# carsonmw3/wavelet-compression

Hardware: AMD Instinct MI355X
Metric: fp64 cells/s, fwd transform+threshold+pack, keep=0.999 (higher is better)
Workload: dtype f64; 1 GPU; c2: 1024 x 64^3 fp64 boxes per GPU, 1 component, keep 0.999, wc_forward (payload bytes identical to the reference's serialize()); boxes_per_gpu=1024, global_batch=1024, parallelism=box-sharded x1

## Files before the change

wavelet-compression_amd/csrc/wc_capi.cpp:

```cpp
#include "wc_ctx.h"

#include <algorithm>
#include <cmath>
#include <cstring>
#include <string>
#include <vector>

using namespace wc;

namespace {

int stage_transform(wc_ctx* c, const void* d_cells, int dtype, double keep, bool sparse) {
    Plan& P = c->plan;
    const UnitDev* du = (const UnitDev*)P.d_units.p;
    const XTile* dxt = (const XTile*)P.d_xtiles.p;
    hipError_t e = hipSuccess;
    if ((e = hipMemsetAsync(c->state.p, 0, P.state_bytes, c->stream)) != hipSuccess)
        return hip_fail(c, e, "memset state");
    unsigned long long* key = (unsigned long long*)((uint8_t*)c->state.p + 16);
    const size_t n = P.units.size();
    uint32_t* spos = (uint32_t*)((uint8_t*)c->state.p + 16 + 12 * n);
    float* coef = (float*)c->coef.p;
    uint8_t* flags = sparse && P.any_sparse ? (uint8_t*)c->flags.p : nullptr;
    {
        StageTimer t(c, WC_STAGE_TRANSFORM);
        e = launch_transform(c->stream, d_cells, dtype, du, dxt, P.ngen, P.lds_gen, coef, 0, key);
        if (e == hipSuccess)
            e = launch_transform_fast(c->stream, d_cells, dtype, du, dxt + P.ngen, P.nfast, P.lds_fast, coef, 0,
                                      key, flags, spos, keep, persistent_grid(c, 0, P.lds_fast));
        if (e == hipSuccess && flags)
            e = launch_transform_fallback(c->stream, d_cells, dtype, du, (int)P.units.size(), dxt, P.lds_fast, coef,
                                          key, spos, keep);
    }
    c->sparse_staged = flags != nullptr;
    return e == hipSuccess ? WC_OK : hip_fail(c, e, "transform launch");
}

int stage_emit(wc_ctx* c, int n, double keep, const float* gthresh, uint8_t* d_payload, uint64_t* d_offsets,
               uint32_t* d_kept, uint2* d_rows = nullptr, const float* d_uthresh = nullptr) {
    Plan& P = c->plan;
    uint8_t* st = (uint8_t*)c->state.p;
    EmitParams p{};
    p.units = (const UnitDev*)P.d_units.p;
    p.edesc = (const EmitDesc*)P.d_edesc.p;
    p.n = n;
    p.ordered = use_ordered(c) ? (c->opt_reverse ? 2u : 1u) : 0u;
    p.key = (const unsigned long long*)(st + 16);
    p.tickets = (uint32_t*)(st + 16 + 8ull * n);
    p.status = (unsigned long long*)(st + round_up(16 + 20ull * n, 8));
    p.payload = d_payload;
    p.offsets = d_offsets;
    p.kept = d_kept;
    p.err = (uint32_t*)c->errflag.p;
    p.keep = keep;
    if (gthresh) {
        p.use_gthresh = 1;
        p.gthresh = *gthresh;
    }
    p.flags = (c->sparse_staged && !gthresh && !d_uthresh) ? (const uint8_t*)c->flags.p : nullptr;
    p.rowinfo = d_rows;
    p.uthresh = d_uthresh;
    StageTimer t(c, WC_STAGE_EMIT);
    hipError_t e = launch_emit(c->stream, p, (const float*)c->coef.p, P.nedesc_small,
                               (uint32_t)P.edesc.size() - P.nedesc_small);
    if (e != hipSuccess) return hip_fail(c, e, "emit launch");
    return WC_OK;
}

int forward_staged(wc_ctx* c, const void* d_cells, int dtype, int n, double keep, uint8_t* d_payload,
                   uint64_t* d_offsets, uint32_t* d_kept, uint2* d_rows = nullptr) {
    int rc = stage_transform(c, d_cells, dtype, keep, c->opt_sparse);
    return rc ? rc : stage_emit(c, n, keep, nullptr, d_payload, d_offsets, d_kept, d_rows);
}

int pin_begin(wc_ctx* c, size_t in_bytes, size_t dev_bytes, uint8_t** pin) {
    int rc;
    hipError_t e;
    if ((rc = ensure(c, c->tol_in, dev_bytes))) return rc;
    if (!c->tol_ev && (e = hipEventCreateWithFlags(&c->tol_ev, hipEventDisableTiming)) != hipSuccess)
        return hip_fail(c, e, "event");
    if (c->tol_ev_live && (e = hipEventSynchronize(c->tol_ev)) != hipSuccess) return hip_fail(c, e, "pinned upload");
    c->tol_ev_live = false;
    if (c->tol_pin_bytes < in_bytes) {
        if (c->tol_pin) (void)hipHostFree(c->tol_pin);
        c->tol_pin = nullptr;
        c->tol_pin_bytes = 0;
        const size_t want = std::max(in_bytes, size_t(4096));
        if ((e = hipHostMalloc(&c->tol_pin, want, hipHostMallocDefault)) != hipSuccess) {
            c->tol_pin = nullptr;
            return fail(c, WC_ERR_NOMEM, std::string("pinned block: ") + hipGetErrorString(e));
        }
        c->tol_pin_bytes = want;
    }
    *pin = (uint8_t*)c->tol_pin;
    return WC_OK;
}

int pin_upload(wc_ctx* c, size_t in_bytes) {
    hipError_t e;
    if ((e = hipMemcpyAsync(c->tol_in.p, c->tol_pin, in_bytes, hipMemcpyHostToDevice, c->stream)) != hipSuccess ||
        (e = hipEventRecord(c->tol_ev, c->stream)) != hipSuccess)
        return hip_fail(c, e, "pinned upload");
    c->tol_ev_live = true;
    return WC_OK;
}

int stage_tol(wc_ctx* c, int n, const double* tol, float* d_thresh, double* d_bound, const float** uthresh) {
    const Plan& P = c->plan;
    const uint32_t solo = (uint32_t)c->opt_tol_solo;
    const uint32_t chunk = std::min<uint32_t>(solo, 8);
    std::vector<uint32_t> slot(n), split;
    std::vector<uint2> items;
    for (int u = 0; u < n; ++u) {
        const uint32_t nt = P.units[u].nftiles;
        if (nt <= solo) {
            slot[u] = 0xffffffffu;
            continue;
        }
        slot[u] = (uint32_t)split.size();
        split.push_back((uint32_t)u);
        for (uint32_t t = 0; t < nt; t += chunk) items.push_back(make_uint2((uint32_t)u, t));
    }
    const size_t nsplit = split.size(), nitems = items.size();
    const size_t o_items = sizeof(double) * n, o_slot = o_items + sizeof(uint2) * nitems, o_split = o_slot + 4ull * n,
                 in_bytes = o_split + 4 * nsplit, o_thresh = round_up(in_bytes, 8);
    int rc;
    hipError_t e;
    uint8_t* pin = nullptr;
    if ((nsplit && (rc = ensure(c, c->tol_bins, sizeof(uint32_t) * WC_HIST_BINS * nsplit))) ||
        (rc = pin_begin(c, in_bytes, o_thresh + sizeof(float) * n, &pin)))
        return rc;
    std::memcpy(pin, tol, sizeof(double) * n);
    if (nitems) std::memcpy(pin + o_items, items.data(), sizeof(uint2) * nitems);
    std::memcpy(pin + o_slot, slot.data(), 4ull * n);
    if (nsplit) std::memcpy(pin + o_split, split.data(), 4 * nsplit);
    if ((rc = pin_upload(c, in_bytes))) return rc;
    uint8_t* d = (uint8_t*)c->tol_in.p;
    if (nsplit && (e = hipMemsetAsync(c->tol_bins.p, 0, sizeof(uint32_t) * WC_HIST_BINS * nsplit, c->stream)) !=
                      hipSuccess)
        return hip_fail(c, e, "memset bins");
    float* th = d_thresh ? d_thresh : (float*)(d + o_thresh);
    StageTimer t(c, WC_STAGE_TOL);
    e = launch_tol(c->stream, (const UnitDev*)P.d_units.p, n, (const uint32_t*)(d + o_slot),
                   (const uint2*)(d + o_items), (uint32_t)nitems, chunk, (const uint32_t*)(d + o_split),
                   (uint32_t)nsplit, (const float*)c->coef.p, (uint32_t*)c->tol_bins.p, (const double*)d, th, d_bound);
    if (e != hipSuccess) return hip_fail(c, e, "tolerance launch");
    *uthresh = th;
    return WC_OK;
}

struct LevelWork {
    const int32_t* levels = nullptr;
    const uint2* hdr = nullptr;
    const uint2* key = nullptr;
    const uint2* lv[WC_MAX_LEVELS - 1] = {};
    uint32_t nhdr = 0, nkey = 0, nlv[WC_MAX_LEVELS - 1] = {};
    int maxl = 1;
};
constexpr uint32_t kLevelKeyChunk = 8;

int upload_levels(wc_ctx* c, int n, const int32_t* levels, LevelWork* w, const void* extra = nullptr,
                  size_t extra_bytes = 0, const void** d_extra = nullptr) {
    const Plan& P = c->plan;
    std::vector<uint2> hdr, key, lv[WC_MAX_LEVELS - 1];
    const uint32_t cb = level_chunk_blocks();
    for (int u = 0; u < n; ++u) {
        const int L = levels[u];
        if (L < 2) continue;
        w->maxl = std::max(w->maxl, L);
        hdr.push_back(make_uint2((uint32_t)u, (uint32_t)L));
        const UnitDev& d = P.units[u];
        for (uint32_t t = 0; t < d.nftiles; t += kLevelKeyChunk) key.push_back(make_uint2((uint32_t)u, t));
        for (int l = 2; l <= L; ++l) {
            const uint64_t nblk = d.ncells >> (3 * l);
            for (uint64_t b = 0; b < nblk; b += cb) lv[l - 2].push_back(make_uint2((uint32_t)u, (uint32_t)(b / cb)));
        }
    }
    size_t items = hdr.size() + key.size();
    for (const auto& v : lv) items += v.size();
    const size_t o_levels = sizeof(uint2) * items, o_extra = round_up(o_levels + sizeof(int32_t) * n, 8),
                 in_bytes = extra_bytes ? o_extra + extra_bytes : o_levels + sizeof(int32_t) * n;
    int rc;
    uint8_t* pin = nullptr;
    if ((rc = pin_begin(c, in_bytes, in_bytes, &pin))) return rc;
    const uint8_t* d = (const uint8_t*)c->tol_in.p;
    size_t o = 0;
    auto put = [&](const std::vector<uint2>& v, const uint2** dev, uint32_t* count) {
        if (!v.empty()) std::memcpy(pin + o, v.data(), sizeof(uint2) * v.size());
        *dev = (const uint2*)(d + o);
        *count = (uint32_t)v.size();
        o += sizeof(uint2) * v.size();
    };
    put(hdr, &w->hdr, &w->nhdr);
    put(key, &w->key, &w->nkey);
    for (int i = 0; i < WC_MAX_LEVELS - 1; ++i) put(lv[i], &w->lv[i], &w->nlv[i]);
    std::memcpy(pin + o_levels, levels, sizeof(int32_t) * n);
    w->levels = (const int32_t*)(d + o_levels);
    if (extra_bytes) {
        std::memcpy(pin + o_extra, extra, extra_bytes);
        *d_extra = d + o_extra;
    }
    if ((rc = ensure(c, c->lv_side, sizeof(float) * (P.coef_extent / 8 + 64)))) return rc;
    return pin_upload(c, in_bytes);
}

int run_levels(wc_ctx* c, const LevelWork& w, bool fwd, bool with_key, const uint32_t* bad = nullptr) {
    const UnitDev* du = (const UnitDev*)c->plan.d_units.p;
    float* coef = (float*)c->coef.p;
    float* side = (float*)c->lv_side.p;
    unsigned long long* key = (unsigned long long*)((uint8_t*)c->state.p + 16);
    StageTimer t(c, WC_STAGE_LEVELS);
    hipError_t e = hipSuccess;
    if (fwd) {
        for (int l = 2; l <= w.maxl && e == hipSuccess; ++l)
            e = launch_level(c->stream, true, du, w.lv[l - 2], w.nlv[l - 2], l - 1, coef, side,
                             with_key && l == 2 ? key : nullptr, nullptr);
        if (e == hipSuccess && with_key) e = launch_level_key(c->stream, du, w.key, w.nkey, kLevelKeyChunk, coef, key);
    } else {
        for (int l = w.maxl; l >= 2 && e == hipSuccess; --l)
            e = launch_level(c->stream, false, du, w.lv[l - 2], w.nlv[l - 2], l - 1, coef, side, nullptr, bad);
    }
    return e == hipSuccess ? WC_OK : hip_fail(c, e, "level pass launch");
}

bool single_level(const int32_t* levels, int n) {
    for (int i = 0; i < n; ++i)
        if (levels[i] != 1) return false;
    return true;
}

}

extern "C" {

const char* wc_version(void) { return "wavelet_amd 0.2 (gfx950; fp-contract=off, no denormal flush)"; }

int wc_device_count(void) {
    int ndev = 0;
    return hipGetDeviceCount(&ndev) == hipSuccess ? ndev : 0;
}

int wc_ctx_create(int device, wc_ctx** out) {
    if (!out) return WC_ERR_INVALID;
    *out = nullptr;
    int ndev = 0;
    if (hipGetDeviceCount(&ndev) != hipSuccess || ndev == 0) return WC_ERR_HIP;
    if (device < 0 || device >= ndev) return WC_ERR_INVALID;
    wc_ctx* c = new wc_ctx();
    c->device = device;
    if (set_device(c) != WC_OK) {
        delete c;
        return WC_ERR_HIP;
    }
    if (hipStreamCreateWithFlags(&c->own, hipStreamNonBlocking) != hipSuccess) {
        delete c;
        return WC_ERR_HIP;
    }
    c->stream = c->own;
    if (ensure(c, c->errflag, 16) != WC_OK || hipMemset(c->errflag.p, 0, 16) != hipSuccess) {
        wc_ctx_destroy(c);
        return WC_ERR_NOMEM;
    }
    *out = c;
    return WC_OK;
}

void wc_ctx_destroy(wc_ctx* c) {
    if (!c) return;
    (void)hipSetDevice(c->device);
    (void)hipStreamSynchronize(c->stream);
    if (c->aux) (void)hipStreamSynchronize(c->aux);
    DevBuf* bufs[] = {&c->coef,          &c->part,           &c->errflag,        &c->state,
                      &c->flags,         &c->h_cells,        &c->h_payload,      &c->h_packed,
                      &c->h_offsets,     &c->h_poff,         &c->h_kept,         &c->h_out,
                      &c->h_rows,        &c->h_rmse,
                      &c->plan.d_units,  &c->plan.d_xtiles,  &c->plan.d_ftiles,  &c->plan.d_dtiles,
                      &c->plan.d_edesc, &c->plan.d_ixtiles, &c->plan.d_rtiles,
                      &c->plan.d_rdtiles, &c->rowinfo,    &c->istate,        &c->npairs,
                      &c->tol_in,        &c->tol_bins,       &c->h_thresh,       &c->h_bound,
                      &c->lv_side};
    for (DevBuf* b : bufs)
        if (b->p) (void)hipFree(b->p);
    for (Plan& P : c->plan_cache) free_plan(P);
    for (hipEvent_t e : c->hev) (void)hipEventDestroy(e);
    for (hipEvent_t e : c->iev) (void)hipEventDestroy(e);
    if (c->aux) (void)hipStreamDestroy(c->aux);
    if (c->up) (void)hipStreamDestroy(c->up);
    if (c->down) (void)hipStreamDestroy(c->down);
    if (c->pinned) (void)hipHostFree(c->pinned);
    if (c->bounce) (void)hipHostFree(c->bounce);
    if (c->tol_pin) (void)hipHostFree(c->tol_pin);
    if (c->tol_ev) (void)hipEventDestroy(c->tol_ev);
    for (hipEvent_t e : c->bev) (void)hipEventDestroy(e);
    for (auto& m : c->marks) {
        c->ev_pool.push_back(m.a);
        c->ev_pool.push_back(m.b);
    }
    for (hipEvent_t e : c->ev_pool) (void)hipEventDestroy(e);
    if (c->own) (void)hipStreamDestroy(c->own);
    delete c;
}

const char* wc_last_error(const wc_ctx* c) { return c ? c->err.c_str() : "null context"; }

int wc_set_stream(wc_ctx* c, void* s) {
    if (!c) return WC_ERR_INVALID;
    hipStream_t next = s ? (hipStream_t)s : c->own;
    hipError_t e = hipSuccess;
    if (next != c->stream) e = hipStreamSynchronize(c->stream);
    c->stream = next;
    return e == hipSuccess ? WC_OK : hip_fail(c, e, "wc_set_stream: synchronize the previous stream");
}

int wc_set_option(wc_ctx* c, int option, int64_t value) {
    if (!c) return WC_ERR_INVALID;
    switch (option) {
        case WC_OPT_SPARSE:
            c->opt_sparse = value != 0;
            return WC_OK;
        case WC_OPT_RIX_XCD:
            c->opt_rix_xcd = value != 0;
            return WC_OK;
        case WC_OPT_INV_GROUPS:
            if (value < 1 || value > 16) return fail(c, WC_ERR_INVALID, "WC_OPT_INV_GROUPS: 1..16");
            c->opt_inv_groups = (int)value;
            return WC_OK;
        case WC_OPT_ORDERED:
            c->opt_ordered = value != 0;
            return WC_OK;
        case WC_OPT_INVERSE_ROWS:
            c->opt_inv_rows = value != 0;
            return WC_OK;
        case WC_OPT_RIX_LDS:
            if (value < 1024 || value > 16384) return fail(c, WC_ERR_INVALID, "WC_OPT_RIX_LDS: 1024..16384 floats");
            c->opt_rix_lds = (int)value;
            return WC_OK;
        case WC_OPT_RIX_BLOCKED:
            c->opt_rix_blocked = value != 0;
            return WC_OK;
        case WC_OPT_RIX_TX:
            if (value < 0 || value > 5) return fail(c, WC_ERR_INVALID, "WC_OPT_RIX_TX: log2 of 1..32 blocks");
            c->opt_rix_lx = (int)value;
            return WC_OK;
        case WC_OPT_HOST_CHUNK:
            if (value < 0) return fail(c, WC_ERR_INVALID, "WC_OPT_HOST_CHUNK: cells >= 0");
            c->opt_host_chunk = value;
            return WC_OK;
        case WC_OPT_SPIN_LIMIT: {
            if (value < 0 || value > 0xffffffffll) return fail(c, WC_ERR_INVALID, "WC_OPT_SPIN_LIMIT: 0..2^32-1 polls");
            hipError_t e;
            if ((e = hipSetDevice(c->device)) != hipSuccess ||
                (e = hipMemsetD32Async((hipDeviceptr_t)((uint32_t*)c->errflag.p + 1), (int)(uint32_t)value, 1,
                                       c->stream)) != hipSuccess)
                return hip_fail(c, e, "WC_OPT_SPIN_LIMIT");
            c->opt_spin_limit = (uint32_t)value;
            return WC_OK;
        }
        case WC_OPT_TICKETS:
            c->force_tickets = value != 0;
            return WC_OK;
        case WC_OPT_REVERSE_TILES:
            c->opt_reverse = value != 0;
            return WC_OK;
        case WC_OPT_HOST_THREADS:
            if (value < -1 || value > 256) return fail(c, WC_ERR_INVALID, "WC_OPT_HOST_THREADS: -1..256");
            c->opt_host_threads = (int)value;
            return WC_OK;
        case WC_OPT_HOST_THP:
            c->opt_host_thp = value != 0;
            return WC_OK;
        case WC_OPT_TOL_SOLO_TILES:
            if (value < 1 || value > (int64_t(1) << 19))
                return fail(c, WC_ERR_INVALID, "WC_OPT_TOL_SOLO_TILES: 1..2^19 flat tiles");
            c->opt_tol_solo = (int)value;
            return WC_OK;
        default:
            return fail(c, WC_ERR_INVALID, "unknown option");
    }
}

int wc_get_option(const wc_ctx* c, int option, int64_t* value) {
    if (!c || !value) return WC_ERR_INVALID;
    switch (option) {
        case WC_OPT_SPARSE: *value = c->opt_sparse; return WC_OK;
        case WC_OPT_RIX_XCD: *value = c->opt_rix_xcd; return WC_OK;
        case WC_OPT_INV_GROUPS: *value = c->opt_inv_groups; return WC_OK;
        case WC_OPT_ORDERED: *value = use_ordered(c) ? 1 : 0; return WC_OK;
        case WC_OPT_INVERSE_ROWS: *value = c->opt_inv_rows; return WC_OK;
        case WC_OPT_RIX_LDS: *value = c->opt_rix_lds; return WC_OK;
        case WC_OPT_RIX_TX: *value = c->opt_rix_lx; return WC_OK;
        case WC_OPT_RIX_BLOCKED: *value = c->opt_rix_blocked; return WC_OK;
        case WC_OPT_HOST_CHUNK: *value = c->opt_host_chunk; return WC_OK;
        case WC_OPT_SPIN_LIMIT: *value = c->opt_spin_limit; return WC_OK;
        case WC_OPT_TICKETS: *value = c->force_tickets ? 1 : 0; return WC_OK;
        case WC_OPT_REVERSE_TILES: *value = c->opt_reverse ? 1 : 0; return WC_OK;
        case WC_OPT_HOST_THREADS:
            *value = c->opt_host_threads < 0 ? host_threads_default() : c->opt_host_threads;
            return WC_OK;
        case WC_OPT_HOST_THP: *value = c->opt_host_thp; return WC_OK;
        case WC_OPT_TOL_SOLO_TILES: *value = c->opt_tol_solo; return WC_OK;
        default: return WC_ERR_INVALID;
    }
}

int wc_synchronize(wc_ctx* c) {
    if (!c) return WC_ERR_INVALID;
    hipError_t e = hipStreamSynchronize(c->stream);
    if (e == hipSuccess && c->aux) e = hipStreamSynchronize(c->aux);
    if (e != hipSuccess) return hip_fail(c, e, "hipStreamSynchronize");
    return check_kernel_errors(c);
}

int wc_forward(wc_ctx* c, const void* d_cells, int dtype, const wc_unit* units, int n, double keep,
               uint8_t* d_payload, uint64_t cap, uint64_t* d_offsets, uint32_t* d_kept) {
    if (!c) return WC_ERR_INVALID;
    int rc;
    if ((rc = validate_units(c, units, n))) return rc;
    if (dtype != WC_F32 && dtype != WC_F64) return fail(c, WC_ERR_INVALID, "dtype");
    if (n == 0) return WC_OK;
    if (!d_cells || !d_payload || !d_offsets || !d_kept) return fail(c, WC_ERR_INVALID, "null buffer");
    if (cap < wc_payload_bound(units, n)) return fail(c, WC_ERR_INVALID, "payload_capacity < wc_payload_bound");
    if ((rc = check_aligned(c, d_cells, "cells")) || (rc = check_aligned(c, d_payload, "payload")) ||
        (rc = check_aligned(c, d_offsets, "offsets", 8)) || (rc = check_aligned(c, d_kept, "kept", 4)))
        return rc;
    if ((rc = set_device(c)) || (rc = get_plan(c, units, n))) return rc;
    if ((rc = ensure_scratch(c))) return rc;
    return forward_staged(c, d_cells, dtype, n, keep, d_payload, d_offsets, d_kept);
}

int wc_forward_rows(wc_ctx* c, const void* d_cells, int dtype, const wc_unit* units, int n, double keep,
                    uint8_t* d_payload, uint64_t cap, uint64_t* d_offsets, uint32_t* d_kept, void* d_rowinfo,
                    uint64_t rowinfo_capacity) {
    if (!c) return WC_ERR_INVALID;
    int rc;
    if ((rc = validate_units(c, units, n))) return rc;
    if (dtype != WC_F32 && dtype != WC_F64) return fail(c, WC_ERR_INVALID, "dtype");
    if (n == 0) return WC_OK;
    if (!d_cells || !d_payload || !d_offsets || !d_kept || !d_rowinfo) return fail(c, WC_ERR_INVALID, "null buffer");
    if (cap < wc_payload_bound(units, n)) return fail(c, WC_ERR_INVALID, "payload_capacity < wc_payload_bound");
    if (rowinfo_capacity < wc_rowindex_bytes(units, n))
        return fail(c, WC_ERR_INVALID, "rowinfo_capacity < wc_rowindex_bytes");
    if ((rc = check_aligned(c, d_cells, "cells")) || (rc = check_aligned(c, d_payload, "payload")) ||
        (rc = check_aligned(c, d_offsets, "offsets", 8)) || (rc = check_aligned(c, d_kept, "kept", 4)) ||
        (rc = check_aligned(c, d_rowinfo, "rowinfo", 8)))
        return rc;
    if ((rc = set_device(c)) || (rc = get_plan(c, units, n))) return rc;
    if (c->plan.rowinfo_entries > 0xffffffffull)
        return fail(c, WC_ERR_INVALID, "wc_forward_rows: more than 2^32 row-index entries in one batch");
    if ((rc = ensure_scratch(c))) return rc;
    return forward_staged(c, d_cells, dtype, n, keep, d_payload, d_offsets, d_kept, (uint2*)d_rowinfo);
}

int wc_forward_stage(wc_ctx* c, const void* d_cells, int dtype, const wc_unit* units, int n, uint64_t* d_hist) {
    if (!c) return WC_ERR_INVALID;
    int rc;
    if ((rc = validate_units(c, units, n))) return rc;
    if (dtype != WC_F32 && dtype != WC_F64) return fail(c, WC_ERR_INVALID, "dtype");
    if (n == 0) return WC_OK;
    if (!d_cells) return fail(c, WC_ERR_INVALID, "null buffer");
    if ((rc = check_aligned(c, d_cells, "cells"))) return rc;
    if ((rc = set_device(c)) || (rc = get_plan(c, units, n))) return rc;
    if ((rc = ensure_scratch(c))) return rc;
    if (!d_hist) {
        if ((rc = stage_transform(c, d_cells, dtype, 0.0, false))) return rc;
        c->staged = true;
        return WC_OK;
    }
    Plan& P = c->plan;
    const UnitDev* du = (const UnitDev*)P.d_units.p;
    const XTile* dxt = (const XTile*)P.d_xtiles.p;
    unsigned long long* key = (unsigned long long*)((uint8_t*)c->state.p + 16);
    float* coef = (float*)c->coef.p;
    hipError_t e = hipMemsetAsync(c->state.p, 0, P.state_bytes, c->stream);
    if (e != hipSuccess) return hip_fail(c, e, "memset state");
    {
        StageTimer t(c, WC_STAGE_TRANSFORM);
        e = launch_transform(c->stream, d_cells, dtype, du, dxt, P.ngen, P.lds_gen, coef, 0, key);
        if (e == hipSuccess)
            e = launch_transform_hist(c->stream, d_cells, dtype, du, dxt + P.ngen, P.nfast, P.lds_fast, coef, key,
                                      (unsigned long long*)d_hist,
                                      persistent_grid(c, 2, transform_hist_lds_bytes(P.lds_fast)));
        if (e != hipSuccess) return hip_fail(c, e, "transform launch");
    }
    c->sparse_staged = false;
    if (P.ngen) {
        const uint32_t max_blocks = 2048;
        StageTimer t(c, WC_STAGE_HIST);
        e = launch_hist(c->stream, du, (const FTile*)P.d_ftiles.p, (uint32_t)P.ftiles.size(), coef, max_blocks,
                        (unsigned long long*)d_hist, true);
        if (e != hipSuccess) return hip_fail(c, e, "histogram launch");
    }
    c->staged = true;
    return WC_OK;
}

int wc_hist_threshold(const uint64_t* hist, double quantile, float* thresh, uint64_t* retained) {
    if (!hist || !thresh || !(quantile >= 0.0 && quantile <= 1.0)) return WC_ERR_INVALID;
    uint64_t total = 0;
    for (int b = 0; b < WC_HIST_BINS; ++b) total += hist[b];
    const uint64_t drop = (uint64_t)std::floor(quantile * (double)total);
    const uint64_t target = total - std::min(drop, total);
    uint64_t cum = 0;
    int bstar = -1;
    if (target > 0)
        for (int b = WC_HIST_BINS - 1; b >= 0; --b) {
            cum += hist[b];
            if (cum >= target) {
                bstar = b;
                break;
            }
        }
    float t;
    if (bstar < 0) {
        t = __builtin_inff();
        cum = 0;
    } else if (bstar == 0) {
        t = -1.0f;
    } else {
        const uint32_t bits = ((uint32_t)bstar << WC_HIST_SHIFT) - 1u;
        std::memcpy(&t, &bits, 4);
    }
    *thresh = t;
    if (retained) *retained = cum;
    return WC_OK;
}

int wc_forward_emit(wc_ctx* c, const wc_unit* units, int n, double keep, const float* thresh, uint8_t* d_payload,
                    uint64_t cap, uint64_t* d_offsets, uint32_t* d_kept) {
    if (!c) return WC_ERR_INVALID;
    int rc;
    if ((rc = validate_units(c, units, n))) return rc;
    if (n == 0) return WC_OK;
    if (!d_payload || !d_offsets || !d_kept) return fail(c, WC_ERR_INVALID, "null buffer");
    if (cap < wc_payload_bound(units, n)) return fail(c, WC_ERR_INVALID, "payload_capacity < wc_payload_bound");
    if ((rc = check_aligned(c, d_payload, "payload")) || (rc = check_aligned(c, d_offsets, "offsets", 8)) ||
        (rc = check_aligned(c, d_kept, "kept", 4)))
        return rc;
    const bool staged = c->staged;
    const uint64_t gen = c->plan_gen;
    if ((rc = set_device(c)) || (rc = get_plan(c, units, n))) return rc;
    if (!staged || gen != c->plan_gen)
        return fail(c, WC_ERR_INVALID, "wc_forward_emit: no staged coefficients for these units (wc_forward_stage)");
    const Plan& P = c->plan;
    const size_t st_off = 16 + 8ull * n;
    hipError_t e = hipMemsetAsync((uint8_t*)c->state.p + st_off, 0, P.state_bytes - st_off, c->stream);
    if (e != hipSuccess) return hip_fail(c, e, "memset status");
    if ((rc = stage_emit(c, n, keep, thresh, d_payload, d_offsets, d_kept))) return rc;
    c->staged = true;
    return WC_OK;
}

int wc_forward_tol(wc_ctx* c, const void* d_cells, int dtype, const wc_unit* units, int n, const double* tol,
                   uint8_t* d_payload, uint64_t cap, uint64_t* d_offsets, uint32_t* d_kept, float* d_thresh,
                   double* d_bound) {
    if (!c) return WC_ERR_INVALID;
    int rc;
    if ((rc = validate_units(c, units, n))) return rc;
    if (dtype != WC_F32 && dtype != WC_F64) return fail(c, WC_ERR_INVALID, "dtype");
    if (n == 0) return WC_OK;
    if (!d_cells || !d_payload || !d_offsets || !d_kept) return fail(c, WC_ERR_INVALID, "null buffer");
    if ((rc = validate_tol(c, units, n, tol))) return rc;
    if (cap < wc_payload_bound(units, n)) return fail(c, WC_ERR_INVALID, "payload_capacity < wc_payload_bound");
    if ((rc = check_aligned(c, d_cells, "cells")) || (rc = check_aligned(c, d_payload, "payload")) ||
        (rc = check_aligned(c, d_offsets, "offsets", 8)) || (rc = check_aligned(c, d_kept, "kept", 4)) ||
        (rc = check_aligned(c, d_thresh, "thresh", 4)) || (rc = check_aligned(c, d_bound, "bound", 8)))
        return rc;
    if ((rc = set_device(c)) || (rc = get_plan(c, units, n))) return rc;
    if ((rc = ensure_scratch(c))) return rc;
    const float* uth = nullptr;
    if ((rc = stage_transform(c, d_cells, dtype, 0.0, false)) || (rc = stage_tol(c, n, tol, d_thresh, d_bound, &uth)))
        return rc;
    return stage_emit(c, n, 0.0, nullptr, d_payload, d_offsets, d_kept, nullptr, uth);
}

int wc_forward_emit_tol(wc_ctx* c, const wc_unit* units, int n, const double* tol, uint8_t* d_payload, uint64_t cap,
                        uint64_t* d_offsets, uint32_t* d_kept, float* d_thresh, double* d_bound) {
    if (!c) return WC_ERR_INVALID;
    int rc;
    if ((rc = validate_units(c, units, n))) return rc;
    if (n == 0) return WC_OK;
    if (!d_payload || !d_offsets || !d_kept) return fail(c, WC_ERR_INVALID, "null buffer");
    if ((rc = validate_tol(c, units, n, tol))) return rc;
    if (cap < wc_payload_bound(units, n)) return fail(c, WC_ERR_INVALID, "payload_capacity < wc_payload_bound");
// ... 462 lines not shown
```

wavelet-compression_amd/csrc/wc_ctx.h:

```cpp
#pragma once

#include "wavelet_amd.h"
#include "wc_hostmem.h"
#include "wc_internal.h"

#include <cstdint>
#include <map>
#include <memory>
#include <string>
#include <utility>
#include <vector>

namespace wc {

size_t transform_lds_bytes(int lbx, int lby, int lbz);
size_t transform_fast_lds_bytes(int lbx, int lby, int lbz);
hipError_t launch_transform(hipStream_t, const void*, int, const UnitDev*, const XTile*, uint32_t, size_t,
                            float*, int, unsigned long long*);
hipError_t launch_transform_fast(hipStream_t, const void*, int, const UnitDev*, const XTile*, uint32_t, size_t,
                                 float*, int, unsigned long long*, uint8_t*, uint32_t*, double, uint32_t);
uint32_t transform_pf_grid(size_t lds);
size_t transform_hist_lds_bytes(size_t lds_fast);
uint32_t transform_hist_grid(size_t lds);
hipError_t launch_transform_hist(hipStream_t, const void*, int, const UnitDev*, const XTile*, uint32_t, size_t,
                                 float*, unsigned long long*, unsigned long long*, uint32_t);
uint32_t inverse_rows_grid(size_t lds);
hipError_t launch_transform_fallback(hipStream_t, const void*, int, const UnitDev*, int, const XTile*, size_t, float*,
                                     const unsigned long long*, const uint32_t*, double);
hipError_t launch_pack(hipStream_t, const UnitDev*, int, const uint32_t*, const uint8_t*, uint64_t*, uint8_t*);
hipError_t launch_decode(hipStream_t, const UnitDev*, const FTile*, uint32_t, const FTile*, uint32_t,
                         unsigned long long*, uint32_t, const uint8_t*, const uint64_t*, uint32_t*,
                         unsigned long long*, float*, uint2*, uint32_t*, int, uint32_t*,
                         const int32_t* levels = nullptr);
hipError_t launch_pair_counts(hipStream_t, const UnitDev*, int, const uint8_t*, const uint64_t*, uint32_t*, uint32_t*);
hipError_t launch_inverse_rows(hipStream_t, const RTile*, uint32_t, size_t, uint32_t, const uint8_t*,
                               const uint64_t*, const uint2*, float*, int, const void*, int, const UnitDev*, int,
                               double*, double*, bool, const uint32_t*);
hipError_t launch_inverse(hipStream_t, const float*, int, const UnitDev*, const XTile*, uint32_t, size_t, uint32_t,
                          size_t, float*, const uint32_t* bad = nullptr);
hipError_t launch_rmse(hipStream_t, const void*, int, const float*, const UnitDev*, int, const FTile*,
                       uint32_t, double*, double*);
hipError_t launch_emit(hipStream_t, const EmitParams&, const float*, uint32_t, uint32_t);
hipError_t launch_hist(hipStream_t, const UnitDev*, const FTile*, uint32_t, const float*, uint32_t,
                       unsigned long long*, bool);
hipError_t launch_tol(hipStream_t, const UnitDev*, int, const uint32_t*, const uint2*, uint32_t, uint32_t,
                      const uint32_t*, uint32_t, const float*, uint32_t*, const double*, float*, double*);
hipError_t launch_level(hipStream_t, bool fwd, const UnitDev*, const uint2* items, uint32_t nitems, int shift,
                        float* coef, float* side, unsigned long long* key, const uint32_t* bad);
hipError_t launch_level_key(hipStream_t, const UnitDev*, const uint2* items, uint32_t nitems, uint32_t chunk,
                            const float* coef, unsigned long long* key);
hipError_t launch_level_headers(hipStream_t, const UnitDev*, const uint2* items, uint32_t nitems, uint8_t* payload);
hipError_t launch_level_flat(hipStream_t, const UnitDev*, const FTile*, uint32_t ntiles, float* coef, float* flat,
                             int to_flat);
uint32_t level_chunk_blocks();
hipError_t launch_decode_corner(hipStream_t, const CornerDesc*, const FTile* dtiles, uint32_t ndt,
                                const uint8_t* payload, const uint64_t* offsets, uint32_t* ticket,
                                unsigned long long* status, float* corner, uint32_t* err, int ordered, uint32_t* bad);
hipError_t launch_corner_box(hipStream_t, const CornerDesc*, const FTile* ftiles, uint32_t nft, const float* corner,
                             float* out, const uint32_t* bad);

struct DevBuf {
    void* p = nullptr;
    size_t bytes = 0;
};

struct Plan {
    std::vector<wc_unit> key;
    std::vector<UnitDev> units;
    std::vector<XTile> xtiles;
    std::vector<XTile> ixtiles;
    std::vector<RTile> rtiles;
    std::vector<FTile> ftiles, dtiles, rdtiles;
    int rix_lds = kRixLds;
    int rix_lx = 4;
    bool rix_xcd = false;
    int inv_groups = 1;
    std::vector<uint32_t> ig_rd, ig_rt;
    std::vector<EmitDesc> edesc;
    uint32_t nedesc_small = 0;
    uint32_t ngen = 0, nfast = 0, netiles = 0;
    uint32_t ign = 0, ifast = 0;
    bool inv_rows = true;
    uint64_t rowinfo_entries = 0;
    size_t lds_rows = 0;
    bool any_sparse = false;
    uint64_t coef_extent = 0;
    uint64_t flag_bytes = 0;
    size_t lds_gen = 0, lds_fast = 0, lds_inverse = 0;
    size_t state_bytes = 0;
    DevBuf d_units, d_xtiles, d_ftiles, d_dtiles, d_edesc, d_ixtiles, d_rtiles, d_rdtiles;
};

inline int ceil_log2(int64_t v) {
    int l = 0;
    while ((int64_t(1) << l) < v) ++l;
    return l;
}

inline uint64_t round_up(uint64_t v, uint64_t m) { return (v + m - 1) / m * m; }

}

using wc::kRixLds;

struct wc_ctx {
    int device = 0;
    hipStream_t own = nullptr;
    hipStream_t stream = nullptr;
    std::string err;
    wc::Plan plan;
    bool plan_valid = false;
    bool opt_ordered = true;
    bool force_tickets = false;
    bool opt_reverse = false;
    uint32_t opt_spin_limit = 0;
    bool opt_sparse = true;
    bool opt_inv_rows = true;
    int opt_rix_lds = kRixLds;
    int opt_rix_lx = 4;
    bool opt_rix_blocked = false;
    bool opt_rix_xcd = false;
    int opt_inv_groups = 1;
    hipStream_t aux = nullptr;
    std::vector<hipEvent_t> iev;
    bool err_check_pending = false;
    bool staged = false;
    bool sparse_staged = false;
    uint64_t plan_gen = 0;
    wc::DevBuf coef, part, errflag, state, flags, rowinfo, npairs;
    wc::DevBuf istate;
    uint32_t epoch = 0;
    wc::DevBuf h_cells, h_payload, h_packed, h_offsets, h_poff, h_kept, h_out;
    wc::DevBuf h_rows, h_rmse;
    int64_t opt_host_chunk = int64_t(1) << 25;
    hipStream_t up = nullptr, down = nullptr;
    std::vector<hipEvent_t> hev;
    void* pinned = nullptr;
    size_t pinned_bytes = 0;
    int opt_host_threads = -1;
    bool opt_host_thp = false;
    int opt_tol_solo = 64;
    void* tol_pin = nullptr;
    size_t tol_pin_bytes = 0;
    hipEvent_t tol_ev = nullptr;
    bool tol_ev_live = false;
    wc::DevBuf tol_in;
    wc::DevBuf tol_bins;
    wc::DevBuf h_thresh, h_bound;
    wc::DevBuf lv_side;
    std::unique_ptr<wc::HostPool> hpool;
    std::unique_ptr<wc::HostPool> upool;
    void* bounce = nullptr;
    std::vector<hipEvent_t> bev;
    std::vector<bool> bev_live;
    uint32_t bnext = 0;
    std::vector<wc::Plan> plan_cache;
    std::map<std::pair<int, size_t>, uint32_t> grids;
    bool prof = false;
    std::vector<hipEvent_t> ev_pool;
    struct Mark {
        int stage;
        hipEvent_t a, b;
    };
    std::vector<Mark> marks;
};

namespace wc {

int fail(wc_ctx* c, int code, const std::string& msg);
int hip_fail(wc_ctx* c, hipError_t e, const char* what);
int ensure(wc_ctx* c, DevBuf& b, size_t bytes);
int validate_units(wc_ctx* c, const wc_unit* units, int n);
int check_aligned(wc_ctx* c, const void* p, const char* what, uintptr_t align = 16);
hipEvent_t take_event(wc_ctx* c);
int upload(wc_ctx* c, DevBuf& d, const void* h, size_t bytes, const char* what);
int set_device(wc_ctx* c);
bool use_ordered(const wc_ctx* c);
int check_kernel_errors(wc_ctx* c);
uint64_t cells_extent(const wc_unit* units, int n);

int get_plan(wc_ctx* c, const wc_unit* units, int n);
void free_plan(Plan& P);
size_t decode_state_bytes(const Plan& P);
int ensure_scratch(wc_ctx* c);
uint32_t persistent_grid(wc_ctx* c, int which, size_t lds);
int inverse_stream(wc_ctx* c, int nev);

int host_threads_default();

int validate_tol(wc_ctx* c, const wc_unit* units, int n, const double* tol);

int validate_levels(wc_ctx* c, const wc_unit* units, int n, const int32_t* levels);
std::vector<int> level_runs(const wc_ctx* c, const wc_unit* units, int n);

int validate_coarse(wc_ctx* c, const wc_unit* units, int n, const int32_t* levels, const int32_t* reduce,
                    const wc_unit* out_units);
uint64_t rows_magic(int32_t d);

struct StageTimer {
    wc_ctx* c;
    int stage;
    hipEvent_t a = nullptr;
    StageTimer(wc_ctx* c_, int s) : c(c_), stage(s) {
        if (c->prof) {
            a = take_event(c);
            (void)hipEventRecord(a, c->stream);
        }
    }
    ~StageTimer() {
        if (c->prof && a) {
            hipEvent_t b = take_event(c);
            (void)hipEventRecord(b, c->stream);
            c->marks.push_back({stage, a, b});
        }
    }
};

}
```

wavelet-compression_amd/csrc/wc_emit.hip:

```cpp
#include "wc_emit.h"

namespace wc {

#ifndef WC_EMIT_MINB
#define WC_EMIT_MINB 8
#endif
#ifndef WC_EMIT_MINB_ROWS
#define WC_EMIT_MINB_ROWS 7
#endif
#ifndef WC_EMIT_MINB8
#define WC_EMIT_MINB8 2
#endif
template <int EW, bool ROWS>
__global__ __launch_bounds__(EW * kWave, EW == 8 ? WC_EMIT_MINB8 : (ROWS ? WC_EMIT_MINB_ROWS : WC_EMIT_MINB)) void k_emit(EmitParams P,
                                                                           const float* __restrict__ coef) {
    __shared__ __attribute__((aligned(16))) uint32_t sm[32];
    __shared__ uint2 stage_all[EW][256 * WC_EMIT_SB];
    const int tid = threadIdx.x;
    uint2* stage = stage_all[tid >> 6];
    const EmitDesc E = P.edesc[blockIdx.x];
    if (P.ordered) {
        emit_tile<EW, ROWS>(P, PlainSrc{coef}, E, P.ordered == 2 ? E.net - 1u - E.index : E.index, sm, stage, tid);
        return;
    }
    if (tid == 0) sm[31] = atomicAdd(P.tickets + E.unit, 1u);
    __syncthreads();
    const uint32_t index = __builtin_amdgcn_readfirstlane(sm[31]);
    emit_tile<EW, ROWS>(P, PlainSrc{coef}, E, index, sm, stage, tid);
}

hipError_t launch_emit(hipStream_t st, const EmitParams& p, const float* coef, uint32_t nsmall, uint32_t nbig) {
    static_assert(kEmitTile == WC_EMIT_EW * 2048 && kEmitTileBig == 8 * 2048, "emit tile sizes");
    EmitParams q = p;
    q.edesc = p.edesc + nsmall;
    if (p.rowinfo) {
        if (nsmall) k_emit<WC_EMIT_EW, true><<<nsmall, WC_EMIT_EW * kWave, 0, st>>>(p, coef);
        if (nbig) k_emit<8, true><<<nbig, 8 * kWave, 0, st>>>(q, coef);
    } else {
        if (nsmall) k_emit<WC_EMIT_EW, false><<<nsmall, WC_EMIT_EW * kWave, 0, st>>>(p, coef);
        if (nbig) k_emit<8, false><<<nbig, 8 * kWave, 0, st>>>(q, coef);
    }
    return hipGetLastError();
}

}
```

wavelet-compression_amd/csrc/wc_internal.h:

```cpp
#pragma once

#include <hip/hip_runtime.h>
#include <stdint.h>

namespace wc {

constexpr int kThreads = 256;
constexpr int kWave = 64;
constexpr int kMaxTileBlocks = 1024;
constexpr int kFlatTile = 4096;
constexpr int kFlatPerThread = kFlatTile / kThreads;

struct UnitDev {
    uint64_t cell_off;
    uint64_t coef_off;
    uint64_t ncells;
    int32_t nx, ny, nz;
    int32_t hx, hy, hz;
    int32_t nbx, nby, nbz;
    int32_t lbx, lby, lbz;
    uint32_t ftile_begin;
    uint32_t nftiles;
    uint64_t pay_off;
    int32_t ntz;
    int32_t fast;
    uint32_t ntx;
    uint32_t xt_begin;
    uint32_t et_begin;
    uint32_t net;
    uint32_t sparse;
    uint32_t dt_begin;
    uint32_t ndt;
    int32_t rix;
    int32_t ilbx, ilby;
    uint64_t row_off;
    uint32_t rt_begin;
    uint32_t nrt;
    uint64_t dmagic;
    uint64_t flag_off;
};

struct XTile {
    uint32_t unit;
    uint32_t bx0, by0, bz0;
};

struct RTile {
    uint64_t row_off;
    uint64_t cell_off;
    uint32_t unit;
    int32_t bx0, by0;
    int32_t W, H, D;
    int32_t lbx, lby;
    int32_t tyv;
    uint32_t nat;
};

#ifndef WC_RIX_RSPAD
#define WC_RIX_RSPAD 4
#endif
#ifndef WC_RIX_WRPAD
#define WC_RIX_WRPAD 16
#endif
__host__ __device__ inline int rix_rs(int lby, int D) { return (D << lby) + WC_RIX_RSPAD; }
__host__ __device__ inline int rix_wr(int lbx, int lby, int D) { return (rix_rs(lby, D) << lbx) + WC_RIX_WRPAD; }

struct FTile {
    uint32_t unit;
    uint32_t index;
};

struct CornerDesc {
    uint64_t dst_off;
    uint64_t out_off;
    uint64_t dmagic;
    uint64_t hmagic;
    int32_t W, H, D;
    int32_t want;
    uint32_t w, h, d;
    uint32_t end;
    uint32_t dt_begin;
    uint32_t direct;
};
static_assert(sizeof(CornerDesc) == 72, "descriptor of 8-B members first");

constexpr uint32_t kCornerRun = 0u;
constexpr uint32_t kCornerRefused = 1u;
constexpr uint32_t kCornerBox = 2u;

constexpr unsigned long long kKeyNaNFirst = ~0ull;

constexpr uint32_t kErrHeader = 1u;
constexpr uint32_t kErrNegativeRun = 2u;

constexpr uint32_t kEpochMask = 0x3fffffffu;

#ifndef WC_EMIT_EW
#define WC_EMIT_EW 4
#endif
constexpr int kEmitTile = WC_EMIT_EW * 2048;
constexpr int kEmitTileBig = 16384;
constexpr uint64_t kEmitBigCells = uint64_t(1) << 21;

struct EmitDesc {
    uint64_t coef_off;
    uint64_t pay_off;
    uint32_t ncells;
    uint32_t unit;
    uint32_t index;
    uint32_t et_begin;
    uint32_t net;
    int32_t nx, ny, nz;
    uint32_t mode;
    uint32_t flag_off;
    uint32_t row_off;
    uint32_t dmul;
};
static_assert(sizeof(EmitDesc) == 64, "one 64-B descriptor per emit block (one scalar load)");

struct EmitParams {
    const UnitDev* units;
    const EmitDesc* edesc;
    int n;
    uint32_t ordered;
    uint32_t* tickets;
    const unsigned long long* key;
    unsigned long long* status;
    uint8_t* payload;
    uint64_t* offsets;
    uint32_t* kept;
    uint32_t* err;
    double keep;
    uint32_t use_gthresh;
    float gthresh;
    const uint8_t* flags;
    uint2* rowinfo;
    const float* uthresh;
};

constexpr int kSegShift = 4;
__host__ __device__ inline uint64_t flag_pos(uint64_t s, int sh) {
    const int lb = 11 - sh, lg = 8 - sh;
    const uint64_t sw = s & ((1ull << lb) - 1);
    return (s & ~((1ull << lb) - 1)) | ((sw & ((1ull << lg) - 1)) << 3) | (sw >> lg);
}
__host__ __device__ inline uint32_t flag_pos32(uint32_t s, int sh) {
    const int lb = 11 - sh, lg = 8 - sh;
    const uint32_t sw = s & ((1u << lb) - 1);
    return (s & ~((1u << lb) - 1)) | ((sw & ((1u << lg) - 1)) << 3) | (sw >> lg);
}
#ifndef WC_RIX_TILE
#define WC_RIX_TILE 4096
#endif
constexpr int kRixTile = WC_RIX_TILE;
constexpr int kRixRounds5 = kRixTile / kThreads;
constexpr int kRixLds = 9216;

}
```

Measured before the change: 430.9 billion cells/s.

## Double-buffer forward state and clear idle half inside emit kernel

Replaces the per-call hipMemsetAsync of the forward state with two alternating state halves. The idle half is zeroed by the emit kernel's blocks after they finish their tiles, so the next call finds it clean. This removes a separate memset launch from the critical path each call. In exchange it adds state memory, dirty-size bookkeeping, and extra stores in the emit kernel.

```diff
diff --git a/wavelet-compression_amd/csrc/wc_capi.cpp b/wavelet-compression_amd/csrc/wc_capi.cpp
--- a/wavelet-compression_amd/csrc/wc_capi.cpp
+++ b/wavelet-compression_amd/csrc/wc_capi.cpp
@@ -10,16 +10,17 @@
 
 namespace {
 
-int stage_transform(wc_ctx* c, const void* d_cells, int dtype, double keep, bool sparse) {
+int stage_transform(wc_ctx* c, const void* d_cells, int dtype, double keep, bool sparse, uint8_t* fst = nullptr) {
     Plan& P = c->plan;
     const UnitDev* du = (const UnitDev*)P.d_units.p;
     const XTile* dxt = (const XTile*)P.d_xtiles.p;
     hipError_t e = hipSuccess;
-    if ((e = hipMemsetAsync(c->state.p, 0, P.state_bytes, c->stream)) != hipSuccess)
+    uint8_t* st = fst ? fst : (uint8_t*)c->state.p;
+    if (!fst && (e = hipMemsetAsync(st, 0, P.state_bytes, c->stream)) != hipSuccess)
         return hip_fail(c, e, "memset state");
-    unsigned long long* key = (unsigned long long*)((uint8_t*)c->state.p + 16);
+    unsigned long long* key = (unsigned long long*)(st + 16);
     const size_t n = P.units.size();
-    uint32_t* spos = (uint32_t*)((uint8_t*)c->state.p + 16 + 12 * n);
+    uint32_t* spos = (uint32_t*)(st + 16 + 12 * n);
     float* coef = (float*)c->coef.p;
     uint8_t* flags = sparse && P.any_sparse ? (uint8_t*)c->flags.p : nullptr;
     {
@@ -37,10 +38,13 @@
 }
 
 int stage_emit(wc_ctx* c, int n, double keep, const float* gthresh, uint8_t* d_payload, uint64_t* d_offsets,
-               uint32_t* d_kept, uint2* d_rows = nullptr, const float* d_uthresh = nullptr) {
+               uint32_t* d_kept, uint2* d_rows = nullptr, const float* d_uthresh = nullptr, uint8_t* fst = nullptr,
+               uint8_t* clr = nullptr, size_t clr_bytes = 0) {
     Plan& P = c->plan;
-    uint8_t* st = (uint8_t*)c->state.p;
+    uint8_t* st = fst ? fst : (uint8_t*)c->state.p;
     EmitParams p{};
+    p.clear = clr;
+    p.clear_n16 = (uint32_t)(clr_bytes / 16);
     p.units = (const UnitDev*)P.d_units.p;
     p.edesc = (const EmitDesc*)P.d_edesc.p;
     p.n = n;
@@ -69,8 +73,35 @@
 
 int forward_staged(wc_ctx* c, const void* d_cells, int dtype, int n, double keep, uint8_t* d_payload,
                    uint64_t* d_offsets, uint32_t* d_kept, uint2* d_rows = nullptr) {
-    int rc = stage_transform(c, d_cells, dtype, keep, c->opt_sparse);
-    return rc ? rc : stage_emit(c, n, keep, nullptr, d_payload, d_offsets, d_kept, d_rows);
+    const Plan& P = c->plan;
+    const size_t need = round_up(P.state_bytes, 16);
+    int rc;
+    if (c->fhalf < need) {
+        c->fhalf = 0;
+        c->fdirty[0] = c->fdirty[1] = wc_ctx::kStateUnknown;
+        if ((rc = ensure(c, c->fstate, 2 * need))) return rc;
+        c->fhalf = (c->fstate.bytes / 2) & ~size_t(15);
+    }
+    const int h = c->fcur, o = h ^ 1;
+    uint8_t* st = (uint8_t*)c->fstate.p + h * c->fhalf;
+    uint8_t* idle = (uint8_t*)c->fstate.p + o * c->fhalf;
+    if (c->fdirty[h]) {
+        const size_t bytes = c->fdirty[h] == wc_ctx::kStateUnknown ? c->fhalf : c->fdirty[h];
+        hipError_t e = hipMemsetAsync(st, 0, bytes, c->stream);
+        if (e != hipSuccess) return hip_fail(c, e, "memset state");
+    }
+    c->fdirty[h] = wc_ctx::kStateUnknown;
+    if ((rc = stage_transform(c, d_cells, dtype, keep, c->opt_sparse, st))) return rc;
+    const size_t dirty = c->fdirty[o];
+    const bool clr = dirty && dirty != wc_ctx::kStateUnknown && dirty / 16 < (1ull << 31) && !P.edesc.empty();
+    if (clr) c->fdirty[o] = wc_ctx::kStateUnknown;
+    if ((rc = stage_emit(c, n, keep, nullptr, d_payload, d_offsets, d_kept, d_rows, nullptr, st, clr ? idle : nullptr,
+                         clr ? dirty : 0)))
+        return rc;
+    if (clr) c->fdirty[o] = 0;
+    c->fdirty[h] = need;
+    c->fcur = o;
+    return WC_OK;
 }
 
 int pin_begin(wc_ctx* c, size_t in_bytes, size_t dev_bytes, uint8_t** pin) {
@@ -278,7 +309,7 @@
                       &c->plan.d_edesc, &c->plan.d_ixtiles, &c->plan.d_rtiles,
                       &c->plan.d_rdtiles, &c->rowinfo,    &c->istate,        &c->npairs,
                       &c->tol_in,        &c->tol_bins,       &c->h_thresh,       &c->h_bound,
-                      &c->lv_side};
+                      &c->lv_side,        &c->fstate};
     for (DevBuf* b : bufs)
         if (b->p) (void)hipFree(b->p);
     for (Plan& P : c->plan_cache) free_plan(P);
diff --git a/wavelet-compression_amd/csrc/wc_ctx.h b/wavelet-compression_amd/csrc/wc_ctx.h
--- a/wavelet-compression_amd/csrc/wc_ctx.h
+++ b/wavelet-compression_amd/csrc/wc_ctx.h
@@ -130,6 +130,11 @@
     wc::DevBuf coef, part, errflag, state, flags, rowinfo, npairs;
     wc::DevBuf istate;
     uint32_t epoch = 0;
+    static constexpr size_t kStateUnknown = ~size_t(0);
+    wc::DevBuf fstate;
+    size_t fhalf = 0;
+    size_t fdirty[2] = {kStateUnknown, kStateUnknown};
+    int fcur = 0;
     wc::DevBuf h_cells, h_payload, h_packed, h_offsets, h_poff, h_kept, h_out;
     wc::DevBuf h_rows, h_rmse;
     int64_t opt_host_chunk = int64_t(1) << 25;
diff --git a/wavelet-compression_amd/csrc/wc_emit.hip b/wavelet-compression_amd/csrc/wc_emit.hip
--- a/wavelet-compression_amd/csrc/wc_emit.hip
+++ b/wavelet-compression_amd/csrc/wc_emit.hip
@@ -1,4 +1,6 @@
 #include "wc_emit.h"
+
+#include <algorithm>
 
 namespace wc {
 
@@ -21,23 +23,31 @@
     const EmitDesc E = P.edesc[blockIdx.x];
     if (P.ordered) {
         emit_tile<EW, ROWS>(P, PlainSrc{coef}, E, P.ordered == 2 ? E.net - 1u - E.index : E.index, sm, stage, tid);
-        return;
+    } else {
+        if (tid == 0) sm[31] = atomicAdd(P.tickets + E.unit, 1u);
+        __syncthreads();
+        const uint32_t index = __builtin_amdgcn_readfirstlane(sm[31]);
+        emit_tile<EW, ROWS>(P, PlainSrc{coef}, E, index, sm, stage, tid);
     }
-    if (tid == 0) sm[31] = atomicAdd(P.tickets + E.unit, 1u);
-    __syncthreads();
-    const uint32_t index = __builtin_amdgcn_readfirstlane(sm[31]);
-    emit_tile<EW, ROWS>(P, PlainSrc{coef}, E, index, sm, stage, tid);
+    if (blockIdx.x < P.clear_blocks)
+        for (uint32_t i = blockIdx.x * (EW * kWave) + tid; i < P.clear_n16; i += P.clear_blocks * (EW * kWave))
+            static_cast<uint4*>(P.clear)[i] = make_uint4(0u, 0u, 0u, 0u);
 }
 
 hipError_t launch_emit(hipStream_t st, const EmitParams& p, const float* coef, uint32_t nsmall, uint32_t nbig) {
     static_assert(kEmitTile == WC_EMIT_EW * 2048 && kEmitTileBig == 8 * 2048, "emit tile sizes");
-    EmitParams q = p;
+    auto clearing = [&p](uint32_t grid, uint32_t threads) {
+        return p.clear ? std::min(grid, (p.clear_n16 + threads - 1) / threads) : 0u;
+    };
+    EmitParams s = p, q = p;
+    s.clear_blocks = clearing(nsmall, WC_EMIT_EW * kWave);
     q.edesc = p.edesc + nsmall;
+    q.clear_blocks = nsmall ? 0u : clearing(nbig, 8 * kWave);
     if (p.rowinfo) {
-        if (nsmall) k_emit<WC_EMIT_EW, true><<<nsmall, WC_EMIT_EW * kWave, 0, st>>>(p, coef);
+        if (nsmall) k_emit<WC_EMIT_EW, true><<<nsmall, WC_EMIT_EW * kWave, 0, st>>>(s, coef);
         if (nbig) k_emit<8, true><<<nbig, 8 * kWave, 0, st>>>(q, coef);
     } else {
-        if (nsmall) k_emit<WC_EMIT_EW, false><<<nsmall, WC_EMIT_EW * kWave, 0, st>>>(p, coef);
+        if (nsmall) k_emit<WC_EMIT_EW, false><<<nsmall, WC_EMIT_EW * kWave, 0, st>>>(s, coef);
         if (nbig) k_emit<8, false><<<nbig, 8 * kWave, 0, st>>>(q, coef);
     }
     return hipGetLastError();
diff --git a/wavelet-compression_amd/csrc/wc_internal.h b/wavelet-compression_amd/csrc/wc_internal.h
--- a/wavelet-compression_amd/csrc/wc_internal.h
+++ b/wavelet-compression_amd/csrc/wc_internal.h
@@ -136,6 +136,9 @@
     const uint8_t* flags;
     uint2* rowinfo;
     const float* uthresh;
+    void* clear;
+    uint32_t clear_n16;
+    uint32_t clear_blocks;
 };
 
 constexpr int kSegShift = 4;
```

New measurement: 430.6 billion cells/s. No clear change (-0.1%).
